# juanmc2005/diart

Hardware: NVIDIA H100
Metric: audio-seconds/sec (real-time factor) at 5s/0.5s step, batch 256 (higher is better)
Workload: dtype f32

## Files before the change

diart_b200/_lib.py:

```python
from __future__ import annotations

import ctypes as C
import os
from typing import Dict, Optional

import numpy as np
import torch

_HERE = os.path.dirname(os.path.abspath(__file__))
LIB_PATH = os.path.join(_HERE, "libdiartb200.so")

_lib: Optional[C.CDLL] = None


class DgTensor(C.Structure):
    _fields_ = [("name", C.c_char_p), ("data", C.c_void_p), ("numel", C.c_int64)]


_P = C.c_void_p
SIGNATURES = {
    "dg_last_error": (C.c_char_p, []),
    "dg_version": (C.c_int, []),
    "dg_launch_count": (C.c_int64, []),
    "dg_profile_enable": (C.c_int, [C.c_int]),
    "dg_profile_report": (C.c_int, [C.c_char_p, C.c_int]),
    "dg_selftest_gemm_tc": (C.c_int, [C.c_int, C.c_int, C.c_int, C.c_int, C.c_int, C.c_int, C.POINTER(C.c_float),
                                      C.POINTER(C.c_float)]),
    "dg_selftest_gemm_tc_grid": (C.c_int, [C.c_int, C.c_int, C.c_int, C.c_int, C.c_int, C.c_int, C.POINTER(C.c_int)]),
    "dg_selftest_gemm_tc_bounds": (C.c_int, [C.c_int, C.c_int, C.c_int, C.c_int, C.POINTER(C.c_int), C.POINTER(C.c_int),
                                             C.POINTER(C.c_int)]),
    "dg_selftest_wgmma_row_shift": (C.c_int, [C.c_int, C.POINTER(C.c_uint)]),
    "dg_selftest_gemm_tc_halo": (C.c_int, [C.c_int, C.c_int, C.c_int, C.c_int, C.c_int, C.c_int, C.POINTER(C.c_int),
                                           C.POINTER(C.c_int)]),
    "dg_selftest_split_f16_host": (C.c_int, [_P, C.c_longlong, _P, _P]),
    "dg_seg_create": (C.c_int, [C.POINTER(DgTensor), C.c_int, C.c_int, C.POINTER(_P)]),
    "dg_seg_dims": (C.c_int, [_P, C.c_int, C.POINTER(C.c_int), C.POINTER(C.c_int)]),
    "dg_seg_set_powerset": (C.c_int, [_P, C.c_int, C.c_int]),
    "dg_seg_forward": (C.c_int, [_P, _P, C.c_int, C.c_int, _P, _P]),
    "dg_seg_destroy": (C.c_int, [_P]),
    "dg_emb_create": (C.c_int, [C.POINTER(DgTensor), C.c_int, C.c_int, C.c_int, C.POINTER(_P)]),
    "dg_emb_dims": (C.c_int, [_P, C.c_int, C.POINTER(C.c_int), C.POINTER(C.c_int)]),
    "dg_emb_forward": (C.c_int, [_P, _P, _P, C.c_int, C.c_int, C.c_int, C.c_int, C.c_int, C.c_float, _P, _P]),
    "dg_emb_forward_rows": (C.c_int, [_P, _P, _P, C.c_int, C.c_int, C.c_int, _P, _P]),
    "dg_emb_destroy": (C.c_int, [_P]),
    "dg_emb_debug_trunk": (C.c_int, [_P, _P, C.c_int, C.c_int, C.c_int, _P, C.c_int64, _P]),
    "dg_seg_debug_stage": (C.c_int, [_P, _P, C.c_int, C.c_int, C.c_int, C.c_int, _P, C.c_int64, _P]),
    "dg_emb_debug_stage": (C.c_int, [_P, _P, _P, C.c_int, C.c_int, C.c_int, C.c_int, C.c_int, C.c_int, _P, C.c_int64, _P]),
    "dg_selftest_sinc_filters_host": (C.c_int, [_P, _P, _P]),
    "dg_osp": (C.c_int, [_P, C.c_int, C.c_int, C.c_int, C.c_float, C.c_float, C.c_int, _P, _P]),
    "dg_normalize_embeddings": (C.c_int, [_P, C.c_int, C.c_int, C.c_float, _P, _P]),
    "dg_cluster_create": (C.c_int, [C.c_int, C.c_int, C.c_double, C.c_double, C.c_double, C.c_int, C.POINTER(_P)]),
    "dg_cluster_set_metric": (C.c_int, [_P, C.c_int]),
    "dg_cluster_step": (C.c_int, [_P, _P, _P, C.c_int, C.c_int, C.c_int, _P, _P, _P]),
    "dg_cluster_reset": (C.c_int, [_P]),
    "dg_cluster_get_state": (C.c_int, [_P, _P, _P, C.POINTER(C.c_int)]),
    "dg_cluster_set_state": (C.c_int, [_P, _P, _P, C.c_int]),
# ... 143 lines not shown
```

diart_b200/csrc/api.cu:

```cuda
#include <math.h>
#include <stdlib.h>
#include <string.h>

#include <map>
#include <sstream>
#include <vector>

#include "host.cuh"

namespace dg {

static thread_local std::string g_err;
std::atomic<long long> g_launches{0};
thread_local int g_sm_limit = 0;
void set_error(const std::string& msg) { g_err = msg; }

struct ProfRec {
  std::string name;
  cudaEvent_t a, b;
};
static bool g_prof = false;
static std::vector<ProfRec> g_recs;
static const bool g_trace = getenv("DG_TRACE_LAUNCHES") && getenv("DG_TRACE_LAUNCHES")[0] == '1';
ProfScope::ProfScope(const char* name_, cudaStream_t st_) : on(g_prof), st(st_), a(nullptr), b(nullptr), name(name_) {
// ... 347 lines not shown
  }
  std::vector<unsigned char> first, cur;
  *equal = 1;
  for (int run = 0; run < 3; run++) {
    DG_CUDA(cudaMemset(dF.p, 0, f32_bytes + 4));
    DG_CUDA(cudaMemset(dOh.p, 0, plane_bytes + 4));
    DG_CUDA(cudaMemset(dOl.p, 0, plane_bytes + 4));
    DG_CUDA(cudaMemset(dPart.p, 0, part_bytes + 4));
    {
      SmLimit cap(run == 1 ? 3 : 0);
      if ((rc = launch_gemm_tc(run == 2 ? ref : t, nullptr))) return rc;
    }
    DG_CUDA(cudaDeviceSynchronize());
    cur.resize(f32_bytes + 2 * plane_bytes + part_bytes);
    DG_CUDA(cudaMemcpy(cur.data(), dF.p, f32_bytes, cudaMemcpyDeviceToHost));
    DG_CUDA(cudaMemcpy(cur.data() + f32_bytes, dOh.p, plane_bytes, cudaMemcpyDeviceToHost));
    DG_CUDA(cudaMemcpy(cur.data() + f32_bytes + plane_bytes, dOl.p, plane_bytes, cudaMemcpyDeviceToHost));
    DG_CUDA(cudaMemcpy(cur.data() + f32_bytes + 2 * plane_bytes, dPart.p, part_bytes, cudaMemcpyDeviceToHost));
    if (run == 0)
      first.swap(cur);
    else if (cur != first)
      *equal = 0;
  }
  return DG_OK;
}

extern "C" int dg_selftest_gemm_tc_bounds(int M, int Cin, int N, int epi, int* outside_unchanged, int* equal, int* refused) {
  const bool planes = epi == 1;
  if (M < 1 || Cin < 64 || Cin % 64 || N < 1 || N % (planes ? 32 : 4) || epi < 0 || epi > 2 || !outside_unchanged || !equal ||
      !refused) {
    set_error("dg_selftest_gemm_tc_bounds: bad arguments");
    return DG_EINVAL;
  }
  const int npad = N <= 64 && epi == 0 ? 64 : (N + 127) / 128 * 128, esize = planes ? 2 : 4;
  const int ldc = N + 40;
  const long long rows = (long long)M + 130;
  uint32_t seed = 4242u;
  auto rnd = [&]() {
    seed = seed * 1664525u + 1013904223u;
    return ((seed >> 8) & 0xFFFF) / 65536.f - 0.5f;
  };
  std::vector<float> A((size_t)M * Cin), Wnk((size_t)N * Cin), bias(N), bsc(N), bsh(N);
  for (auto& v : A) v = 2.f * rnd();
  for (auto& v : Wnk) v = 0.25f * rnd();
  for (int n = 0; n < N; n++) {
    bias[n] = rnd();
// ... 59 lines not shown
```

diart_b200/csrc/dg_common.cuh:

```cuda
#pragma once
#include <cuda_runtime.h>
#include <stdint.h>
#include <stdio.h>

#include <atomic>
#include <string>
#include <vector>

namespace dg {

void set_error(const std::string& msg);
extern std::atomic<long long> g_launches;
extern thread_local int g_sm_limit;
inline int usable_sms() {
  int dev = 0, sms = 132;
  cudaGetDevice(&dev);
  cudaDeviceGetAttribute(&sms, cudaDevAttrMultiProcessorCount, dev);
  return (g_sm_limit > 0 && g_sm_limit < sms) ? g_sm_limit : sms;
}

#define DG_CUDA(expr)                                                                   \
  do {                                                                                  \
    cudaError_t _e = (expr);                                                            \
    if (_e != cudaSuccess) {                                                            \
// ... 100 lines not shown
  float* out_f32;
  void* out_hi;
  void* out_lo;
  int ldc;
  int epi;
  const char* tag;
  const int* tap_off;
  int Wp, Hp, Wop, Hop, stride2, relu;
  const void* res_hi;
  const void* res_lo;
  const float* pool_w;
  float* pool_part;
  int pool_item_rows, pool_K;
  int pool3_T, pool3_tile_rows;
  int tap_boxes;
};
inline int gemm_tc_pool3_tile_rows(int item_rows) {
  for (int t = 126; t >= 96; t -= 3)
    if (item_rows % t == 0) return t;
  return 0;
}
int launch_gemm_tc(const TcGemm& g, cudaStream_t st);
bool gemm_tc_halo(const TcGemm& g);
int selftest_wgmma_row_shift(int base_offset_mode, unsigned* ok_shifts);
int launch_split_ex(const float* x, long long rows_out, int C, int ld_in, int ld_out, int pool, int item_rows,
                    const float* sc, const float* sh, void* hi, void* lo, cudaStream_t st, const int* skip_flag = nullptr);
void split_weights_host(const float* w, int N, int Npad, int K, uint16_t* hi, uint16_t* lo, float scale = 1.f);
float weight_plane_scale(const float* w, size_t n);
uint16_t host_f32_to_h16(float f);
float host_h16_to_f32(uint16_t h);
int sinc_tc_rows_per_item(const Geom& g);
size_t sinc_tc_plane_elems(int B, const Geom& g);
void sinc_tc_pack_filters(const float* filt, uint16_t* planes );
void sinc_tc_affine_consts(const float* filt, float beta, float* cf);
int launch_sinc_prep(const float* wav, const float* mean, const float* rstd, int B, const Geom& g, void* planes_hi,
                     void* planes_lo, cudaStream_t st, const int* skip_flag = nullptr);
int launch_sinc0_tc(float gamma, const float* cf_dev, const void* w_planes, int B, const Geom& g, const void* planes_hi,
                    const void* planes_lo, float* p0, cudaStream_t st, const int* skip_flag = nullptr);
struct SincStreamGeom {
  int Ls;
  int P;
  int rows;
  size_t plane;
};
SincStreamGeom sinc_stream_geom(int B, const Geom& g, int hop);
int launch_overlap_check(const float* wav, int B, int S, int hop, int* flag, cudaStream_t st);
// ... 143 lines not shown
```

diart_b200/csrc/gemm_tc.cu:

```cuda
#include <cuda.h>
#include <cuda_bf16.h>
#include <math.h>
#include <stdlib.h>
#include <string.h>

#include <algorithm>
#include <map>
#include <mutex>
#include <string>
#include <utility>
#include <vector>

#include "dg_common.cuh"
#include "tc_ptx.cuh"

namespace dg {

constexpr int TC_BM = 128, TC_BK = 32, TC_THREADS = 384;
constexpr int TC_SMEM_MAX = 227 * 1024;

struct TcArgs {
  long long M;
  int N;
  int m_tiles, n_tiles;
// ... 3 lines not shown
  const float* bn_shift;
  float* out_f32;
  __nv_bfloat16* out_hi;
  __nv_bfloat16* out_lo;
  int ldc;
  float acc_scale;
  int tap_off[9];
  int Wp, Hp, Wop, Hop, stride2, relu;
  const __nv_bfloat16* res_hi;
  const __nv_bfloat16* res_lo;
  const float* pool_w;
  float* pool_part;
  int pool_item_rows, pool_K;
  int tile_rows, pool3_T;
  unsigned* tile_ctr;
  int halo_rows;
  int cin;
  int wblocks;
  int halo_bytes;
  int op_bytes;
};

enum TcEpi { TC_BIAS_F32 = 0, TC_LEAKY_BN_SPLIT = 1, TC_LEAKY_BN_F32 = 2, TC_CONV2D = 3, TC_POOL = 4, TC_MAXPOOL3 = 5 };

__host__ __device__ constexpr bool tc_pooling(int epi) { return epi == TC_POOL || epi == TC_MAXPOOL3; }
__host__ __device__ constexpr bool tc_box_store(int epi) { return epi == TC_BIAS_F32 || epi == TC_LEAKY_BN_SPLIT || epi == TC_LEAKY_BN_F32; }

template <int BN>
struct TcSmem {
  static constexpr int A_BYTES = TC_BM * TC_BK * 2;
  static constexpr int W_BYTES = BN * TC_BK * 2;
  static constexpr int STAGE_BYTES = 2 * A_BYTES + 2 * W_BYTES;
  static constexpr int W_STAGE_BYTES = 2 * W_BYTES;
  static constexpr int NSTAGE = BN == 128 ? 4 : 6;
  static constexpr int NSTAGE_HALO = BN == 128 ? 5 : 6;
  __host__ static int halo_bytes(int cin, int rows) { return (2 * ((cin + 31) / 32) * rows * 64 + 1023) / 1024 * 1024; }
  __host__ static int halo_op_bytes(int cin, int rows) { return 2 * halo_bytes(cin, rows) + NSTAGE_HALO * W_STAGE_BYTES; }
  static constexpr int BAR_BYTES = 256;
  static constexpr int PARAM_FLOATS = 3 * BN;
  static constexpr int CHUNK_W = 64;
  static constexpr int CHUNK_FLOATS = CHUNK_W / 32 * TC_BM * 33;
  __host__ __device__ static constexpr int extra_floats(int epi) { return epi == TC_POOL ? 128 * 4 + 4 * 2 * 8 * 32 : (epi == TC_MAXPOOL3 ? 4 * 2 * 2 * 32 : 0); }
  __host__ __device__ static constexpr int consumer_floats(int epi) { return PARAM_FLOATS + (tc_pooling(epi) ? CHUNK_FLOATS + extra_floats(epi) : 0); }
  static constexpr int ACC_LD = BN + 4;
  static constexpr int BOX_BYTES = TC_BM * 128;
  __host__ __device__ static constexpr int stage_tile_bytes(int epi) {
    return tc_pooling(epi) ? 0 : (epi == TC_CONV2D ? TC_BM * ACC_LD * 4 : TC_BM * BN * 4);
  }
  __host__ __device__ static constexpr int total(int epi, int op_bytes = NSTAGE * STAGE_BYTES) {
    return op_bytes + stage_tile_bytes(epi) + BAR_BYTES + 2 * consumer_floats(epi) * 4 + 1024;
  }
};
static_assert(TcSmem<128>::total(TC_POOL) <= TC_SMEM_MAX && TcSmem<64>::total(TC_MAXPOOL3) <= TC_SMEM_MAX &&
              TcSmem<128>::total(TC_CONV2D) <= TC_SMEM_MAX && TcSmem<64>::total(TC_CONV2D) <= TC_SMEM_MAX &&
              TcSmem<32>::total(TC_CONV2D) <= TC_SMEM_MAX && TcSmem<128>::total(TC_BIAS_F32) <= TC_SMEM_MAX,
              "gemm_tc: shared memory");

template <int BN, int EPI>
__device__ __forceinline__ void tc_stage_params(const TcArgs& a, float* params, int bar, int n0, int et) {
  named_sync(bar, 128);
  for (int i = et; i < BN; i += 128) {
// ... 272 lines not shown
                }
              }
            }
#pragma unroll
            for (int sg = 0; sg < 2; sg++) {
              stg[((rg * 2 + sg) * 2 + 0) * 32 + col] = s1[sg];
              stg[((rg * 2 + sg) * 2 + 1) * 32 + col] = s2[sg];
            }
          }
          named_sync(bar, 128);
          {
            const int col = et & 31, q = et >> 5, sg = q >> 1, j = q & 1, n = n0 + c + col;
            const float tot = ((stg[((0 * 2 + sg) * 2 + j) * 32 + col] + stg[((1 * 2 + sg) * 2 + j) * 32 + col]) +
                               stg[((2 * 2 + sg) * 2 + j) * 32 + col]) + stg[((3 * 2 + sg) * 2 + j) * 32 + col];
            if (n < a.N) a.pool_part[(((size_t)mt * 2 + sg) * 2 + j) * a.N + n] = tot;
          }
          named_sync(bar, 128);
          continue;
        }
      }
    }
}

template <int BN, int EPI, bool HALO>
__global__ void __launch_bounds__(TC_THREADS, 1)
gemm_tc_kernel(const __grid_constant__ CUtensorMap tmA_hi, const __grid_constant__ CUtensorMap tmA_lo,
               const __grid_constant__ CUtensorMap tmW_hi, const __grid_constant__ CUtensorMap tmW_lo,
               const __grid_constant__ CUtensorMap tmC0, const __grid_constant__ CUtensorMap tmC1, TcArgs a) {
  using S = TcSmem<BN>;
  constexpr bool POOLING = tc_pooling(EPI);
  constexpr int NSTAGE = HALO ? S::NSTAGE_HALO : S::NSTAGE;
  extern __shared__ unsigned char smem_raw[];
  unsigned char* smem = reinterpret_cast<unsigned char*>((reinterpret_cast<uintptr_t>(smem_raw) + 1023) & ~uintptr_t(1023));
  unsigned char* ring = HALO ? smem + 2 * a.halo_bytes : smem;
  constexpr int RING_STAGE = HALO ? S::W_STAGE_BYTES : S::STAGE_BYTES;
  unsigned char* tile_s = smem + a.op_bytes;
  uint64_t* bars = reinterpret_cast<uint64_t*>(tile_s + S::stage_tile_bytes(EPI));
  uint64_t* full = bars;
  uint64_t* empty = bars + NSTAGE;
  uint64_t* tile_full = bars + 2 * NSTAGE;
  uint64_t* tile_empty = tile_full + 2;
  uint64_t* halo_full = tile_empty + 2;
  uint64_t* halo_empty = halo_full + 2;
  volatile int* tile_idx = reinterpret_cast<volatile int*>(halo_empty + 2);
  float* cons = reinterpret_cast<float*>(reinterpret_cast<unsigned char*>(bars) + S::BAR_BYTES);

  const int warp = __shfl_sync(0xffffffffu, (int)(threadIdx.x >> 5), 0), lane = threadIdx.x & 31;
  const int wg = warp >> 2;
  const int num_tiles = a.m_tiles * a.n_tiles;
  const int kblocks = HALO ? a.wblocks : a.KW * a.cin_blocks;
  const int halo_box = a.halo_rows * 64, halo_cb = (a.cin + 31) / 32;

  if (threadIdx.x == 0) {
    for (int s = 0; s < NSTAGE; s++) {
      mbar_init(&full[s], 1);
      mbar_init(&empty[s], 1);
    }
    for (int c = 0; c < 2; c++) {
      mbar_init(&tile_full[c], 1);
      mbar_init(&tile_empty[c], 128);
      mbar_init(&halo_full[c], 1);
      mbar_init(&halo_empty[c], 1);
    }
    asm volatile("fence.mbarrier_init.release.cluster;" ::: "memory");
  }
  __syncthreads();

  if (wg == 0) {
    setmaxnreg_dec<HALO ? 48 : 40>();
    if (threadIdx.x == 0) {
      int stage = 0, phase = 0, next = 0;
      bool halo_next = false;
      for (int i = 0, tile = blockIdx.x;; i++) {
        const int c = i & 1;
        mbar_wait(&tile_empty[c], ((i >> 1) & 1) ^ 1);
        if (tile >= num_tiles) {
          tile_idx[c] = -1;
          mbar_arrive(&tile_full[c]);
          mbar_wait(&tile_empty[c ^ 1], (((i + 1) >> 1) & 1) ^ 1);
          tile_idx[c ^ 1] = -2;
          mbar_arrive(&tile_full[c ^ 1]);
          break;
        }
        tile_idx[c] = tile;
        mbar_arrive(&tile_full[c]);
        const int mt = tile / a.n_tiles, nt = tile - mt * a.n_tiles;
        const int m0 = mt * (EPI == TC_MAXPOOL3 ? a.tile_rows : TC_BM), n0 = nt * BN;
        if constexpr (HALO) {
          auto load_halo = [&](int cc, int r0) {
            unsigned char* hs = smem + cc * a.halo_bytes;
            mbar_expect_tx(&halo_full[cc], 2 * halo_cb * halo_box);
            for (int cb = 0; cb < halo_cb; cb++) {
              tma_load_2d(hs + cb * halo_box, &tmA_hi, cb * TC_BK, r0, &halo_full[cc]);
              tma_load_2d(hs + (halo_cb + cb) * halo_box, &tmA_lo, cb * TC_BK, r0, &halo_full[cc]);
            }
          };
          if (!halo_next) {
            mbar_wait(&halo_empty[c], ((i >> 1) & 1) ^ 1);
            load_halo(c, m0);
          }
          halo_next = false;
          next = POOLING ? (int)gridDim.x + (int)atomicAdd(&a.tile_ctr[0], 1u) : tile + (int)gridDim.x;
          const int next_m0 = next / a.n_tiles * (EPI == TC_MAXPOOL3 ? a.tile_rows : TC_BM);
          const uint32_t next_par = (((i + 1) >> 1) & 1) ^ 1;
          for (int kb = 0; kb < kblocks; kb++) {
            const long long t0 = clock64();
            for (;;) {
              if (!halo_next && next < num_tiles && mbar_test_wait(&halo_empty[c ^ 1], next_par)) {
                load_halo(c ^ 1, next_m0);
                halo_next = true;
              }
              if (mbar_test_wait(&empty[stage], phase ^ 1)) break;
              if (clock64() - t0 > 4000000000LL) __trap();
            }
            unsigned char* st = ring + stage * RING_STAGE;
            mbar_expect_tx(&full[stage], S::W_STAGE_BYTES);
            tma_load_2d(st, &tmW_hi, kb * TC_BK, n0, &full[stage]);
            tma_load_2d(st + S::W_BYTES, &tmW_lo, kb * TC_BK, n0, &full[stage]);
            if (++stage == NSTAGE) {
              stage = 0;
              phase ^= 1;
            }
          }
        }
        for (int j = 0; j < (HALO ? 0 : a.KW); j++) {
          for (int cb = 0; cb < a.cin_blocks; cb++) {
            mbar_wait(&empty[stage], phase ^ 1);
            unsigned char* st = smem + stage * S::STAGE_BYTES;
            mbar_expect_tx(&full[stage], S::STAGE_BYTES);
            const int kcol = (j * a.cin_blocks + cb) * TC_BK;
            tma_load_2d(st, &tmA_hi, cb * TC_BK, m0 + a.tap_off[j], &full[stage]);
            tma_load_2d(st + S::A_BYTES, &tmA_lo, cb * TC_BK, m0 + a.tap_off[j], &full[stage]);
            tma_load_2d(st + 2 * S::A_BYTES, &tmW_hi, kcol, n0, &full[stage]);
            tma_load_2d(st + 2 * S::A_BYTES + S::W_BYTES, &tmW_lo, kcol, n0, &full[stage]);
            if (++stage == NSTAGE) {
              stage = 0;
              phase ^= 1;
            }
          }
        }
        if (!HALO) next = POOLING ? (int)gridDim.x + (int)atomicAdd(&a.tile_ctr[0], 1u) : tile + (int)gridDim.x;
        tile = next;
      }
      if (POOLING) {
        __threadfence();
        if (atomicAdd(&a.tile_ctr[1], 1u) == gridDim.x - 1) {
          atomicExch(&a.tile_ctr[0], 0u);
          atomicExch(&a.tile_ctr[1], 0u);
        }
      }
    }
    return;
  }
  setmaxnreg_inc<HALO ? 224 : 232>();
  const int c = wg - 1, quad = warp & 3, et = threadIdx.x - 128 * wg;
  float* params = cons + c * S::consumer_floats(EPI);
  float* chunk = params + S::PARAM_FLOATS;
  float* pool_stage = chunk + S::CHUNK_FLOATS;
  const int bar = 1 + c, turn = 3 + c, turn_other = 3 + (c ^ 1), acc_free = 5 + c, acc_free_other = 5 + (c ^ 1);
  if (c == 1) {
    named_arrive(3, 256);
    if (!POOLING) named_arrive(5, 256);
  }
  for (int n = 0;; n++) {
    mbar_wait(&tile_full[c], n & 1);
    const int tile = tile_idx[c];
    mbar_arrive(&tile_empty[c]);
    if (tc_box_store(EPI) && tile >= 0 && (a.n_tiles > 1 || n == 0))
      tc_stage_params<BN, EPI>(a, params, bar, (tile - tile / a.n_tiles * a.n_tiles) * BN, et);
    named_sync(turn, 256);
    if (tile < 0) {
      if (tile == -1) {
        named_arrive(turn_other, 256);
        if (!POOLING) named_sync(acc_free, 256);
      }
      break;
    }
    const int pos = (2 * n + c) * kblocks;
    int stage = pos % NSTAGE, phase = (pos / NSTAGE) & 1;
    float acc[2][BN / 2];
#pragma unroll
    for (int i = 0; i < BN / 2; i++) acc[0][i] = acc[1][i] = 0.f;
    uint32_t htap = 0;
    int hch = 0;
    if constexpr (HALO) mbar_wait(&halo_full[c], n & 1);
    const uint32_t hs = smem_u32(smem + c * a.halo_bytes);
    for (int kb = 0; kb < kblocks; kb++) {
      mbar_wait(&full[stage], phase);
      const uint32_t sa = smem_u32(ring + stage * RING_STAGE);
      const uint32_t sw = HALO ? sa : sa + 2 * S::A_BYTES;
      const uint64_t w_hi = wg_desc_sw64(sw), w_lo = wg_desc_sw64(sw + S::W_BYTES);
      constexpr uint64_t HALF = (uint64_t)((64 * TC_BK * 2) >> 4);
      wg_fence_acc(acc[0]);
      wg_fence_acc(acc[1]);
      wg_fence();
#pragma unroll
      for (int ks = 0; ks < TC_BK / 16; ks++) {
        const uint64_t adv = (uint64_t)((ks * 32) >> 4);
        uint64_t a_hi, a_lo;
        if constexpr (HALO) {
          const uint32_t aa = hs + (uint32_t)(hch >> 5) * halo_box + (uint32_t)(hch & 31) * 2 + htap;
          a_hi = wg_desc_sw64(aa);
          a_lo = wg_desc_sw64(aa + halo_cb * halo_box);
          hch += 16;
          const bool next_tap = hch == a.cin;
          hch = next_tap ? 0 : hch;
          htap += next_tap ? a.dil * 64 : 0;
        } else {
          a_hi = wg_desc_sw64(sa) + adv;
          a_lo = wg_desc_sw64(sa + S::A_BYTES) + adv;
        }
#pragma unroll
        for (int h = 0; h < 2; h++) {
          wgmma_ss<BN>(acc[h], a_lo + h * HALF, w_hi + adv, (kb | ks) != 0);
          wgmma_ss<BN>(acc[h], a_hi + h * HALF, w_lo + adv, 1);
          wgmma_ss<BN>(acc[h], a_hi + h * HALF, w_hi + adv, 1);
        }
      }
      wg_commit();
      wg_wait<1>();
      wg_fence_acc(acc[0]);
      wg_fence_acc(acc[1]);
      if (kb > 0 && et == 0) mbar_arrive(&empty[stage == 0 ? NSTAGE - 1 : stage - 1]);
      if (++stage == NSTAGE) {
        stage = 0;
        phase ^= 1;
      }
    }
    named_arrive(turn_other, 256);
    wg_wait<0>();
    wg_fence_acc(acc[0]);
    wg_fence_acc(acc[1]);
    if (et == 0) mbar_arrive(&empty[stage == 0 ? NSTAGE - 1 : stage - 1]);
    if (HALO && et == 0) mbar_arrive(&halo_empty[c]);
    const int mt = tile / a.n_tiles, nt = tile - mt * a.n_tiles;
    const bool stage_params = a.n_tiles > 1 || n == 0;
    if constexpr (POOLING) {
      tc_pool_epilogue_tile<BN, EPI>(a, params, chunk, pool_stage, acc, bar, mt, nt * BN, quad, lane, et, stage_params);
    } else if constexpr (EPI == TC_CONV2D) {
      float* acc_s = reinterpret_cast<float*>(tile_s);
      named_sync(acc_free, 256);
#pragma unroll
      for (int h = 0; h < 2; h++) {
        const int r0 = 64 * h + 16 * quad + (lane >> 2);
#pragma unroll
        for (int j = 0; j < BN / 8; j++) {
          const int col = 8 * j + 2 * (lane & 3);
          *reinterpret_cast<float2*>(acc_s + r0 * S::ACC_LD + col) = make_float2(acc[h][4 * j], acc[h][4 * j + 1]);
          *reinterpret_cast<float2*>(acc_s + (r0 + 8) * S::ACC_LD + col) = make_float2(acc[h][4 * j + 2], acc[h][4 * j + 3]);
        }
      }
      named_sync(bar, 128);
      if (stage_params) tc_stage_params<BN, EPI>(a, params, bar, nt * BN, et);
      tc_conv2d_epilogue_tile<BN>(a, params, acc_s + et * S::ACC_LD, mt, nt * BN, quad, lane);
      named_arrive(acc_free_other, 256);
    } else {
      named_sync(acc_free, 256);
// ... 77 lines not shown
  }
  void* base = nullptr;
  if (cudaGetSymbolAddress(&base, g_tc_tile_ctr) != cudaSuccess) {
    set_error("gemm_tc: cannot address the tile counters");
    return nullptr;
  }
  return static_cast<unsigned*>(base) + 2 * slot;
}

static int tc_bn(const TcGemm& g) { return g.epi == TC_MAXPOOL3 || (g.Npad == 64 && g.epi == TC_BIAS_F32) ? 64 : 128; }
static int tc_halo_rows(const TcGemm& g) {
  return (TC_BM + (g.KW - ((g.KW * g.Cin) % 32 ? 0 : 1)) * g.dil + 7) / 8 * 8;
}
template <int BN>
static int tc_halo_smem(const TcGemm& g) { return TcSmem<BN>::total(g.epi, TcSmem<BN>::halo_op_bytes(g.Cin, tc_halo_rows(g))); }

bool gemm_tc_halo(const TcGemm& g) {
  if (g.tap_boxes || g.epi == TC_CONV2D || g.tap_off || g.KW < 2 || g.dil < 1 || g.Cin % 16 || g.Cin > 128 ||
      tc_halo_rows(g) > 256)
    return false;
  return (tc_bn(g) == 64 ? tc_halo_smem<64>(g) : tc_halo_smem<128>(g)) <= TC_SMEM_MAX;
}

static int tc_setup(const TcGemm& g, int bn, int epi, bool halo, CUtensorMap* maps, TcArgs& a) {
  const int Ktot = g.KW * g.Cin, bk = TC_BK, a_rows = halo ? tc_halo_rows(g) : TC_BM;
  if (make_map(&maps[0], g.A_hi, g.Mtot, g.Cin, g.lda, bk, a_rows) || make_map(&maps[1], g.A_lo, g.Mtot, g.Cin, g.lda, bk, a_rows) ||
      make_map(&maps[2], g.W_hi, g.Npad, Ktot, Ktot, bk, bn) || make_map(&maps[3], g.W_lo, g.Npad, Ktot, Ktot, bk, bn))
    return -2;
  memset(&maps[4], 0, 2 * sizeof(CUtensorMap));
  if (epi == TC_LEAKY_BN_SPLIT) {
    if (make_map(&maps[4], g.out_hi, g.M, g.N, g.ldc, 64, TC_BM) || make_map(&maps[5], g.out_lo, g.M, g.N, g.ldc, 64, TC_BM))
      return -2;
  } else if (tc_box_store(epi)) {
    if (make_map(&maps[4], g.out_f32, g.M, g.N, g.ldc, 32, TC_BM, true)) return -2;
  }
  a = TcArgs{};
  a.M = g.M; a.N = g.N; a.n_tiles = (g.N + bn - 1) / bn;
  a.tile_rows = epi == TC_MAXPOOL3 ? g.pool3_tile_rows : TC_BM;
  a.pool3_T = g.pool3_T;
  a.m_tiles = (int)((g.M + a.tile_rows - 1) / a.tile_rows);
  a.KW = g.KW; a.dil = g.dil; a.cin_blocks = g.Cin / bk;
  a.bias = g.bias; a.bn_scale = g.bn_scale; a.bn_shift = g.bn_shift;
  a.out_f32 = g.out_f32; a.out_hi = reinterpret_cast<__nv_bfloat16*>(g.out_hi);
  a.out_lo = reinterpret_cast<__nv_bfloat16*>(g.out_lo); a.ldc = g.ldc;
  a.acc_scale = g.w_scale > 0.f ? 1.f / g.w_scale : 1.f;
  for (int j = 0; j < 9; j++) a.tap_off[j] = j < g.KW ? (g.tap_off ? g.tap_off[j] : j * g.dil) : 0;
  a.Wp = g.Wp; a.Hp = g.Hp; a.Wop = g.Wop; a.Hop = g.Hop; a.stride2 = g.stride2; a.relu = g.relu;
  a.res_hi = reinterpret_cast<const __nv_bfloat16*>(g.res_hi);
  a.res_lo = reinterpret_cast<const __nv_bfloat16*>(g.res_lo);
  a.pool_w = g.pool_w; a.pool_part = g.pool_part; a.pool_item_rows = g.pool_item_rows; a.pool_K = g.pool_K;
  a.cin = g.Cin;
  if (halo) {
    a.halo_rows = a_rows;
    a.wblocks = (Ktot + bk - 1) / bk;
    a.halo_bytes = bn == 64 ? TcSmem<64>::halo_bytes(g.Cin, a_rows) : TcSmem<128>::halo_bytes(g.Cin, a_rows);
    a.op_bytes = bn == 64 ? TcSmem<64>::halo_op_bytes(g.Cin, a_rows) : TcSmem<128>::halo_op_bytes(g.Cin, a_rows);
  } else {
    a.op_bytes = bn == 128 ? TcSmem<128>::NSTAGE * TcSmem<128>::STAGE_BYTES
                           : (bn == 64 ? TcSmem<64>::NSTAGE * TcSmem<64>::STAGE_BYTES : TcSmem<32>::NSTAGE * TcSmem<32>::STAGE_BYTES);
  }
  return 0;
}

static int tc_grid(const TcArgs& a) {
  const int sms = usable_sms();
  const int tiles = a.m_tiles * a.n_tiles;
  return tiles < sms ? tiles : sms;
}

template <int BN, int EPI, bool HALO>
static int launch_tc(const TcGemm& g, cudaStream_t st) {
  using S = TcSmem<BN>;
  CUtensorMap m[6];
  TcArgs a;
  if (tc_setup(g, BN, EPI, HALO, m, a)) return -2;
  if (tc_pooling(EPI) && !(a.tile_ctr = tile_counter(st))) return -2;
  auto kern = gemm_tc_kernel<BN, EPI, HALO>;
  static bool attr_done[64] = {};
  if (first_use_on_device(attr_done))
    DG_CUDA(cudaFuncSetAttribute(kern, cudaFuncAttributeMaxDynamicSharedMemorySize, HALO ? TC_SMEM_MAX : S::total(EPI)));
  kern<<<tc_grid(a), TC_THREADS, S::total(EPI, a.op_bytes), st>>>(m[0], m[1], m[2], m[3], m[4], m[5], a);
  DG_LAUNCHED();
  return 0;
}

template <int BN, int EPI>
static int launch_tc(const TcGemm& g, cudaStream_t st) {
  return gemm_tc_halo(g) ? launch_tc<BN, EPI, true>(g, st) : launch_tc<BN, EPI, false>(g, st);
}

int launch_gemm_tc(const TcGemm& g, cudaStream_t st) {
  ProfScope _ps(g.tag ? g.tag : "gemm_tc", st);
  if (g.Cin % (gemm_tc_halo(g) ? 16 : 64) || g.lda % 8 || g.ldc % (g.epi == TC_LEAKY_BN_SPLIT ? 8 : 4) ||
      (g.Npad % 128 && g.Npad != 64 && g.Npad != 32) || g.KW < 1 || g.KW > 9) {
    set_error("gemm_tc: Cin must be a multiple of 64 (a Conv1d of 2..9 taps over at most 128 channels whose tile halo fits "
              "in shared memory, e.g. Cin 80: a multiple of 16), A pitch a multiple of 8, output pitch a multiple of 4 "
              "(8 for 16-bit planes), padded N 32, 64 or a multiple of 128, at most 9 taps");
    return -1;
  }
  if (g.epi == TC_LEAKY_BN_SPLIT && g.N % 32) {
    set_error("gemm_tc (planes): N must be a multiple of 32");
    return -1;
  }
  if (tc_box_store(g.epi)) {
    const bool planes = g.epi == TC_LEAKY_BN_SPLIT;
    const uintptr_t base = planes ? ((uintptr_t)g.out_hi | (uintptr_t)g.out_lo) : (uintptr_t)g.out_f32;
    if (!base || (planes && (!g.out_hi || !g.out_lo)) || base % 16 || g.ldc < g.N || g.M >= (1LL << 31)) {
      set_error("gemm_tc: the output needs a 16-byte aligned base, a pitch of at least N and fewer than 2^31 rows");
      return -1;
    }
  }
  if (g.epi == TC_CONV2D) {
    if (g.ldc % 32 || g.N % 32 || g.Wp < 3 || g.Hp < 3 || (!g.out_hi && !g.out_f32) || g.M >= (1LL << 31)) {
      set_error("gemm_tc (conv2d): channel counts must be multiples of 32");
      return -1;
    }
    if (g.Npad == 32) return launch_tc<32, TC_CONV2D, false>(g, st);
    if (g.Npad == 64) return launch_tc<64, TC_CONV2D, false>(g, st);
    return launch_tc<128, TC_CONV2D, false>(g, st);
  }
  if (g.epi == TC_POOL) {
    if (g.Npad % 128 || !g.pool_w || !g.pool_part || g.pool_K < 1 || g.pool_K > 4 || g.pool_item_rows < TC_BM) {
      set_error("gemm_tc (pool): needs 128-wide tiles, 1..4 speakers and items of at least 128 rows");
      return -1;
    }
    return launch_tc<128, TC_POOL>(g, st);
  }
  if (g.epi == TC_MAXPOOL3) {
    if (g.Npad != 64 || !g.out_f32 || !g.pool_part || g.pool3_T < 1 || g.pool3_tile_rows < 3 || g.pool3_tile_rows > 126 ||
        g.pool3_tile_rows % 3 || g.pool_item_rows % g.pool3_tile_rows || g.M % g.pool_item_rows) {
      set_error("gemm_tc (maxpool3): needs 64 output channels and tiles of 3..126 rows (a multiple of 3) that divide the item");
      return -1;
    }
    return launch_tc<64, TC_MAXPOOL3>(g, st);
  }
  if (g.Npad == 64 && g.epi == TC_BIAS_F32) return launch_tc<64, TC_BIAS_F32>(g, st);
  switch (g.epi) {
    case TC_BIAS_F32:
      return launch_tc<128, TC_BIAS_F32>(g, st);
    case TC_LEAKY_BN_SPLIT:
      return launch_tc<128, TC_LEAKY_BN_SPLIT>(g, st);
    default:
// ... 198 lines not shown
```

include/diart_b200.h:

```cpp
#ifndef DIART_B200_H
#define DIART_B200_H

#include <stddef.h>
#include <stdint.h>

#ifdef __cplusplus
extern "C" {
#endif

#define DG_OK 0
#define DG_EINVAL (-1)
#define DG_ECUDA (-2)
#define DG_EWEIGHT (-3)
#define DG_ENCCL (-4)

typedef struct dg_tensor {
  const char* name;
  const float* data;
  int64_t numel;
} dg_tensor;

typedef struct dg_seg dg_seg;
typedef struct dg_emb dg_emb;
typedef struct dg_cluster dg_cluster;
// ... 151 lines not shown
int dg_selftest_multi_frames_host(int slots, int max_wps, int out_chunk, int out_step, int n_rates, const int32_t* rates,
                                  int n_ops, const int32_t* ops, int32_t* result, int64_t* records, int cap, int* n_records);
int dg_selftest_multi_staging_host(int slots, int C, int n_ops, const int32_t* ops, const float* samples_host, int32_t* result,
                                   float* rings_host);
int dg_multi_create_vad(dg_seg* seg, int chunk_samples, int step_samples, int max_streams, int max_windows_per_stream,
                        double tau, int num_windows, const double* hamming_host, dg_multi** out);

typedef struct dg_resample dg_resample;
int dg_resample_create(int orig_rate, int new_rate, const float* taps_host, int width, int device, dg_resample** out);
int64_t dg_resample_out_len(const dg_resample* h, int64_t num_samples);
int dg_resample_forward(dg_resample* h, const float* in_dev, int B, int64_t L, float* out_dev, void* stream);
int dg_resample_destroy(dg_resample* h);
int dg_stream_create_resampled(int chunk_samples, int step_samples, dg_resample* rs, int max_windows, int device,
                               dg_stream** out);
int dg_stream_crop_host(dg_stream* h, int n, const int64_t* ranges_host, float* out_host);

int64_t dg_launch_count(void);
int dg_profile_enable(int enable);
int dg_selftest_gemm_tc(int M, int Cin, int KW, int dil, int N, int epi, float* max_abs_diff, float* out_rms);
int dg_selftest_gemm_tc_grid(int M, int Cin, int KW, int dil, int N, int epi, int* equal);
int dg_selftest_gemm_tc_bounds(int M, int Cin, int N, int epi, int* outside_unchanged, int* equal, int* refused);
int dg_selftest_wgmma_row_shift(int base_offset_mode, unsigned* ok_shifts);
int dg_selftest_gemm_tc_halo(int M, int Cin, int KW, int dil, int N, int epi, int* equal, int* halo);
int dg_selftest_split_f16_host(const float* x, long long n, unsigned short* hi, unsigned short* lo);
int dg_selftest_sinc_filters_host(const float* low_hz, const float* band_hz, float* filters);
int dg_profile_report(char* buf, int cap);

int dg_cluster_record_len(const dg_cluster* h);
int dg_cluster_export_delta(dg_cluster* h, double* record_dev, void* stream);
int dg_cluster_merge(dg_cluster* h, const double* records_dev , int world, int rank,
                     int32_t* maps_dev , int n_maps, void* stream);
int dg_pipeline_identity_export(dg_pipeline* h, double* record_dev, void* stream);
int dg_pipeline_identity_merge(dg_pipeline* h, const double* records_dev, int world, int rank, void* stream);

#ifdef __cplusplus
}
#endif
#endif
```

Measured before the change: 23040.

## Add per-channel-block halo A-loading mode to TMA/WGMMA conv GEMM

Adds a third A-operand mode for the tensor-core conv GEMM, used when the full halo tile does not fit in shared memory. Each 32-channel block is loaded once as a halo tile covering all taps into a three-slot ring, and only the weight tiles are streamed per tap. This replaces reloading the A box for every tap, cutting A-side TMA traffic and shared-memory fill per K step. It also switches to an atomic tile counter when the SM count is capped, and adds a selftest comparing the new mode against tap-box loading. The extra barriers and slots add complexity and more shared memory.

```diff
diff --git a/diart_b200/_lib.py b/diart_b200/_lib.py
--- a/diart_b200/_lib.py
+++ b/diart_b200/_lib.py
@@ -32,6 +32,8 @@
     "dg_selftest_wgmma_row_shift": (C.c_int, [C.c_int, C.POINTER(C.c_uint)]),
     "dg_selftest_gemm_tc_halo": (C.c_int, [C.c_int, C.c_int, C.c_int, C.c_int, C.c_int, C.c_int, C.POINTER(C.c_int),
                                            C.POINTER(C.c_int)]),
+    "dg_selftest_gemm_tc_modes": (C.c_int, [C.c_int, C.c_int, C.c_int, C.c_int, C.c_int, C.c_int, C.c_int, C.POINTER(C.c_int),
+                                            C.POINTER(C.c_float), C.POINTER(C.c_float), C.POINTER(C.c_int)]),
     "dg_selftest_split_f16_host": (C.c_int, [_P, C.c_longlong, _P, _P]),
     "dg_seg_create": (C.c_int, [C.POINTER(DgTensor), C.c_int, C.c_int, C.POINTER(_P)]),
     "dg_seg_dims": (C.c_int, [_P, C.c_int, C.POINTER(C.c_int), C.POINTER(C.c_int)]),
diff --git a/diart_b200/csrc/api.cu b/diart_b200/csrc/api.cu
--- a/diart_b200/csrc/api.cu
+++ b/diart_b200/csrc/api.cu
@@ -393,6 +393,98 @@
     else if (cur != first)
       *equal = 0;
   }
+  return DG_OK;
+}
+
+extern "C" int dg_selftest_gemm_tc_modes(int M, int Cin, int KW, int dil, int N, int epi, int shift, int* mode,
+                                         float* max_abs_diff, float* sum_abs, int* shift_equal) {
+  if (M < 1 || Cin < 64 || Cin % 64 || KW < 1 || KW > 9 || dil < 1 || N < 1 || N % 4 || epi < 0 || epi > 2 ||
+      (epi == 1 && N % 32) || shift < 0 || !mode || !max_abs_diff || !sum_abs || !shift_equal) {
+    set_error("dg_selftest_gemm_tc_modes: bad arguments");
+    return DG_EINVAL;
+  }
+  const int K = KW * Cin, npad = N == 64 ? 64 : (N + 127) / 128 * 128;
+  const long long Ms = (long long)M + shift;
+  uint32_t seed = 5151u;
+  auto rnd = [&]() {
+    seed = seed * 1664525u + 1013904223u;
+    return ((seed >> 8) & 0xFFFF) / 65536.f - 0.5f;
+  };
+  std::vector<float> A((size_t)Ms * Cin), Aabs(A.size()), Wnk((size_t)N * K), Wabs_kn((size_t)K * N), bias(N), bsc(N), bsh(N);
+  for (auto& v : A) v = 2.f * rnd();
+  for (auto& v : Wnk) v = 0.25f * rnd();
+  for (int n = 0; n < N; n++) {
+    bias[n] = rnd();
+    bsc[n] = 1.f + rnd();
+    bsh[n] = rnd();
+  }
+  for (size_t i = 0; i < A.size(); i++) Aabs[i] = fabsf(A[i]);
+  for (int n = 0; n < N; n++)
+    for (int k = 0; k < K; k++) Wabs_kn[(size_t)k * N + n] = fabsf(Wnk[(size_t)n * K + k]);
+  const bool planes = epi == 1;
+  const size_t out_bytes = (size_t)Ms * N * (planes ? 2 : 4);
+  DevBuf dA, dAabs, dWabs, dB, dS, dH, dAh, dAl, dSum, dO[3], dOl[3];
+  WeightPlanes dW;
+  if (upload(dA, A) || upload(dAabs, Aabs) || upload(dWabs, Wabs_kn) || upload(dB, bias) || upload(dS, bsc) || upload(dH, bsh) ||
+      upload_split(dW, Wnk, N, npad, K))
+    return DG_ECUDA;
+  if (dAh.ensure((size_t)Ms * Cin * 2) || dAl.ensure((size_t)Ms * Cin * 2) || dSum.ensure((size_t)M * N * 4)) return DG_ECUDA;
+  for (int r = 0; r < 3; r++)
+    if (dO[r].ensure(out_bytes) || dOl[r].ensure(out_bytes)) return DG_ECUDA;
+  int rc;
+  if ((rc = launch_split_ex(dA.as<float>(), Ms, Cin, Cin, Cin, 0, 1, nullptr, nullptr, dAh.p, dAl.p, nullptr))) return rc;
+  const size_t a_off = (size_t)shift * Cin * 2;
+  TcGemm t{};
+  t.A_hi = static_cast<char*>(dAh.p) + a_off; t.A_lo = static_cast<char*>(dAl.p) + a_off; t.lda = Cin; t.Cin = Cin;
+  t.KW = KW; t.dil = dil; t.Mtot = M; t.M = M; t.N = N; t.bias = dB.as<float>(); t.bn_scale = dS.as<float>();
+  t.bn_shift = dH.as<float>(); t.ldc = N; t.epi = epi; t.tag = "selftest_tc_modes";
+  if ((rc = set_weights(t, dW))) return rc;
+  *mode = gemm_tc_halo(t) ? 1 : (gemm_tc_cb_halo(t) ? 2 : 0);
+  TcGemm boxes = t, shifted = t;
+  boxes.tap_boxes = 1;
+  shifted.A_hi = dAh.p; shifted.A_lo = dAl.p; shifted.Mtot = shifted.M = Ms;
+  const TcGemm* runs[3] = {&t, &boxes, &shifted};
+  for (int r = 0; r < 3; r++) {
+    TcGemm g = *runs[r];
+    g.out_f32 = planes ? nullptr : dO[r].as<float>();
+    g.out_hi = planes ? dO[r].p : nullptr;
+    g.out_lo = planes ? dOl[r].p : nullptr;
+    if ((rc = launch_gemm_tc(g, nullptr))) return rc;
+  }
+  GemmArgs s{};
+  s.A = dAabs.as<float>() + (size_t)shift * Cin; s.lda = Cin; s.Cin = Cin; s.KW = KW; s.dil = dil; s.Mtot = M; s.M = M;
+  s.W = dWabs.as<float>(); s.ldw = N; s.N = N; s.C = dSum.as<float>(); s.ldc = N; s.epi = EPI_BIAS; s.tag = "selftest_simt";
+  if ((rc = launch_gemm(s, nullptr))) return rc;
+  DG_CUDA(cudaDeviceSynchronize());
+  std::vector<unsigned char> o[3], ol[3];
+  for (int r = 0; r < 3; r++) {
+    const size_t bytes = (r == 2 ? (size_t)Ms : (size_t)M) * N * (planes ? 2 : 4);
+    o[r].resize(bytes);
+    DG_CUDA(cudaMemcpy(o[r].data(), dO[r].p, bytes, cudaMemcpyDeviceToHost));
+    if (planes) {
+      ol[r].resize(bytes);
+      DG_CUDA(cudaMemcpy(ol[r].data(), dOl[r].p, bytes, cudaMemcpyDeviceToHost));
+    }
+  }
+  auto value = [&](int r, size_t i) {
+    if (!planes) return (double)reinterpret_cast<const float*>(o[r].data())[i];
+    return (double)host_h16_to_f32(reinterpret_cast<const uint16_t*>(o[r].data())[i]) +
+           (double)host_h16_to_f32(reinterpret_cast<const uint16_t*>(ol[r].data())[i]);
+  };
+  std::vector<float> sums((size_t)M * N);
+  DG_CUDA(cudaMemcpy(sums.data(), dSum.p, sums.size() * 4, cudaMemcpyDeviceToHost));
+  double md = 0, ms = 0;
+  for (size_t i = 0; i < (size_t)M * N; i++) {
+    const double d = fabs(value(0, i) - value(1, i));
+    if (!(d <= md)) md = d;
+    const double sg = (double)sums[i] * (epi == 0 ? 1.0 : fabs((double)bsc[i % N]));
+    if (sg > ms) ms = sg;
+  }
+  *max_abs_diff = (float)md;
+  *sum_abs = (float)ms;
+  const size_t row_bytes = (size_t)N * (planes ? 2 : 4), skip = (size_t)shift * row_bytes;
+  *shift_equal = memcmp(o[0].data(), o[2].data() + skip, (size_t)M * row_bytes) == 0 &&
+                 (!planes || memcmp(ol[0].data(), ol[2].data() + skip, (size_t)M * row_bytes) == 0);
   return DG_OK;
 }
 
diff --git a/diart_b200/csrc/dg_common.cuh b/diart_b200/csrc/dg_common.cuh
--- a/diart_b200/csrc/dg_common.cuh
+++ b/diart_b200/csrc/dg_common.cuh
@@ -146,6 +146,7 @@
 }
 int launch_gemm_tc(const TcGemm& g, cudaStream_t st);
 bool gemm_tc_halo(const TcGemm& g);
+bool gemm_tc_cb_halo(const TcGemm& g);
 int selftest_wgmma_row_shift(int base_offset_mode, unsigned* ok_shifts);
 int launch_split_ex(const float* x, long long rows_out, int C, int ld_in, int ld_out, int pool, int item_rows,
                     const float* sc, const float* sh, void* hi, void* lo, cudaStream_t st, const int* skip_flag = nullptr);
diff --git a/diart_b200/csrc/gemm_tc.cu b/diart_b200/csrc/gemm_tc.cu
--- a/diart_b200/csrc/gemm_tc.cu
+++ b/diart_b200/csrc/gemm_tc.cu
@@ -49,6 +49,8 @@
 };
 
 enum TcEpi { TC_BIAS_F32 = 0, TC_LEAKY_BN_SPLIT = 1, TC_LEAKY_BN_F32 = 2, TC_CONV2D = 3, TC_POOL = 4, TC_MAXPOOL3 = 5 };
+enum TcAMode { TC_TAP_BOXES = 0, TC_HALO = 1, TC_CB_HALO = 2 };
+constexpr int TC_CB_SLOTS = 3;
 
 __host__ __device__ constexpr bool tc_pooling(int epi) { return epi == TC_POOL || epi == TC_MAXPOOL3; }
 __host__ __device__ constexpr bool tc_box_store(int epi) { return epi == TC_BIAS_F32 || epi == TC_LEAKY_BN_SPLIT || epi == TC_LEAKY_BN_F32; }
@@ -63,7 +65,10 @@
   static constexpr int NSTAGE_HALO = BN == 128 ? 5 : 6;
   __host__ static int halo_bytes(int cin, int rows) { return (2 * ((cin + 31) / 32) * rows * 64 + 1023) / 1024 * 1024; }
   __host__ static int halo_op_bytes(int cin, int rows) { return 2 * halo_bytes(cin, rows) + NSTAGE_HALO * W_STAGE_BYTES; }
+  static constexpr int NSTAGE_CB = 6;
+  __host__ static int cb_op_bytes(int rows) { return TC_CB_SLOTS * halo_bytes(32, rows) + NSTAGE_CB * W_STAGE_BYTES; }
   static constexpr int BAR_BYTES = 256;
+  static_assert((2 * 6 + 4 + 2 * TC_CB_SLOTS) * 8 + 8 <= BAR_BYTES, "gemm_tc: barrier block");
   static constexpr int PARAM_FLOATS = 3 * BN;
   static constexpr int CHUNK_W = 64;
   static constexpr int CHUNK_FLOATS = CHUNK_W / 32 * TC_BM * 33;
@@ -382,18 +387,19 @@
     }
 }
 
-template <int BN, int EPI, bool HALO>
+template <int BN, int EPI, int AMODE>
 __global__ void __launch_bounds__(TC_THREADS, 1)
 gemm_tc_kernel(const __grid_constant__ CUtensorMap tmA_hi, const __grid_constant__ CUtensorMap tmA_lo,
                const __grid_constant__ CUtensorMap tmW_hi, const __grid_constant__ CUtensorMap tmW_lo,
                const __grid_constant__ CUtensorMap tmC0, const __grid_constant__ CUtensorMap tmC1, TcArgs a) {
   using S = TcSmem<BN>;
   constexpr bool POOLING = tc_pooling(EPI);
-  constexpr int NSTAGE = HALO ? S::NSTAGE_HALO : S::NSTAGE;
+  constexpr bool HALO = AMODE == TC_HALO, CB_HALO = AMODE == TC_CB_HALO;
+  constexpr int NSTAGE = HALO ? S::NSTAGE_HALO : (CB_HALO ? S::NSTAGE_CB : S::NSTAGE);
   extern __shared__ unsigned char smem_raw[];
   unsigned char* smem = reinterpret_cast<unsigned char*>((reinterpret_cast<uintptr_t>(smem_raw) + 1023) & ~uintptr_t(1023));
-  unsigned char* ring = HALO ? smem + 2 * a.halo_bytes : smem;
-  constexpr int RING_STAGE = HALO ? S::W_STAGE_BYTES : S::STAGE_BYTES;
+  unsigned char* ring = smem + (HALO ? 2 : (CB_HALO ? TC_CB_SLOTS : 0)) * a.halo_bytes;
+  constexpr int RING_STAGE = AMODE != TC_TAP_BOXES ? S::W_STAGE_BYTES : S::STAGE_BYTES;
   unsigned char* tile_s = smem + a.op_bytes;
   uint64_t* bars = reinterpret_cast<uint64_t*>(tile_s + S::stage_tile_bytes(EPI));
   uint64_t* full = bars;
@@ -401,8 +407,8 @@
   uint64_t* tile_full = bars + 2 * NSTAGE;
   uint64_t* tile_empty = tile_full + 2;
   uint64_t* halo_full = tile_empty + 2;
-  uint64_t* halo_empty = halo_full + 2;
-  volatile int* tile_idx = reinterpret_cast<volatile int*>(halo_empty + 2);
+  uint64_t* halo_empty = halo_full + TC_CB_SLOTS;
+  volatile int* tile_idx = reinterpret_cast<volatile int*>(halo_empty + TC_CB_SLOTS);
   float* cons = reinterpret_cast<float*>(reinterpret_cast<unsigned char*>(bars) + S::BAR_BYTES);
 
   const int warp = __shfl_sync(0xffffffffu, (int)(threadIdx.x >> 5), 0), lane = threadIdx.x & 31;
@@ -419,17 +425,20 @@
     for (int c = 0; c < 2; c++) {
       mbar_init(&tile_full[c], 1);
       mbar_init(&tile_empty[c], 128);
-      mbar_init(&halo_full[c], 1);
-      mbar_init(&halo_empty[c], 1);
+    }
+    for (int s = 0; s < TC_CB_SLOTS; s++) {
+      mbar_init(&halo_full[s], 1);
+      mbar_init(&halo_empty[s], 1);
     }
     asm volatile("fence.mbarrier_init.release.cluster;" ::: "memory");
   }
   __syncthreads();
 
   if (wg == 0) {
-    setmaxnreg_dec<HALO ? 48 : 40>();
+    setmaxnreg_dec<AMODE != TC_TAP_BOXES ? 48 : 40>();
     if (threadIdx.x == 0) {
       int stage = 0, phase = 0, next = 0;
+      int astage = 0, aphase = 0;
       bool halo_next = false;
       for (int i = 0, tile = blockIdx.x;; i++) {
         const int c = i & 1;
@@ -460,7 +469,7 @@
             load_halo(c, m0);
           }
           halo_next = false;
-          next = POOLING ? (int)gridDim.x + (int)atomicAdd(&a.tile_ctr[0], 1u) : tile + (int)gridDim.x;
+          next = a.tile_ctr ? (int)gridDim.x + (int)atomicAdd(&a.tile_ctr[0], 1u) : tile + (int)gridDim.x;
           const int next_m0 = next / a.n_tiles * (EPI == TC_MAXPOOL3 ? a.tile_rows : TC_BM);
           const uint32_t next_par = (((i + 1) >> 1) & 1) ^ 1;
           for (int kb = 0; kb < kblocks; kb++) {
@@ -483,7 +492,32 @@
             }
           }
         }
-        for (int j = 0; j < (HALO ? 0 : a.KW); j++) {
+        if constexpr (CB_HALO) {
+          for (int cb = 0; cb < a.cin_blocks; cb++) {
+            mbar_wait(&halo_empty[astage], aphase ^ 1);
+            unsigned char* as = smem + astage * a.halo_bytes;
+            mbar_expect_tx(&halo_full[astage], 2 * halo_box);
+            tma_load_2d(as, &tmA_hi, cb * TC_BK, m0, &halo_full[astage]);
+            tma_load_2d(as + halo_box, &tmA_lo, cb * TC_BK, m0, &halo_full[astage]);
+            if (++astage == TC_CB_SLOTS) {
+              astage = 0;
+              aphase ^= 1;
+            }
+            for (int j = 0; j < a.KW; j++) {
+              mbar_wait(&empty[stage], phase ^ 1);
+              unsigned char* st = ring + stage * RING_STAGE;
+              mbar_expect_tx(&full[stage], S::W_STAGE_BYTES);
+              const int kcol = j * a.cin + cb * TC_BK;
+              tma_load_2d(st, &tmW_hi, kcol, n0, &full[stage]);
+              tma_load_2d(st + S::W_BYTES, &tmW_lo, kcol, n0, &full[stage]);
+              if (++stage == NSTAGE) {
+                stage = 0;
+                phase ^= 1;
+              }
+            }
+          }
+        }
+        for (int j = 0; j < (AMODE == TC_TAP_BOXES ? a.KW : 0); j++) {
           for (int cb = 0; cb < a.cin_blocks; cb++) {
             mbar_wait(&empty[stage], phase ^ 1);
             unsigned char* st = smem + stage * S::STAGE_BYTES;
@@ -499,10 +533,10 @@
             }
           }
         }
-        if (!HALO) next = POOLING ? (int)gridDim.x + (int)atomicAdd(&a.tile_ctr[0], 1u) : tile + (int)gridDim.x;
+        if (!HALO) next = a.tile_ctr ? (int)gridDim.x + (int)atomicAdd(&a.tile_ctr[0], 1u) : tile + (int)gridDim.x;
         tile = next;
       }
-      if (POOLING) {
+      if (a.tile_ctr) {
         __threadfence();
         if (atomicAdd(&a.tile_ctr[1], 1u) == gridDim.x - 1) {
           atomicExch(&a.tile_ctr[0], 0u);
@@ -512,7 +546,7 @@
     }
     return;
   }
-  setmaxnreg_inc<HALO ? 224 : 232>();
+  setmaxnreg_inc<AMODE != TC_TAP_BOXES ? 224 : 232>();
   const int c = wg - 1, quad = warp & 3, et = threadIdx.x - 128 * wg;
   float* params = cons + c * S::consumer_floats(EPI);
   float* chunk = params + S::PARAM_FLOATS;
@@ -538,6 +572,8 @@
     }
     const int pos = (2 * n + c) * kblocks;
     int stage = pos % NSTAGE, phase = (pos / NSTAGE) & 1;
+    const int apos = (2 * n + c) * a.cin_blocks;
+    int astage = apos % TC_CB_SLOTS, aphase = (apos / TC_CB_SLOTS) & 1, tap = 0;
     float acc[2][BN / 2];
 #pragma unroll
     for (int i = 0; i < BN / 2; i++) acc[0][i] = acc[1][i] = 0.f;
@@ -546,9 +582,10 @@
     if constexpr (HALO) mbar_wait(&halo_full[c], n & 1);
     const uint32_t hs = smem_u32(smem + c * a.halo_bytes);
     for (int kb = 0; kb < kblocks; kb++) {
+      if constexpr (CB_HALO) mbar_wait(&halo_full[astage], aphase);
       mbar_wait(&full[stage], phase);
       const uint32_t sa = smem_u32(ring + stage * RING_STAGE);
-      const uint32_t sw = HALO ? sa : sa + 2 * S::A_BYTES;
+      const uint32_t sw = AMODE != TC_TAP_BOXES ? sa : sa + 2 * S::A_BYTES;
       const uint64_t w_hi = wg_desc_sw64(sw), w_lo = wg_desc_sw64(sw + S::W_BYTES);
       constexpr uint64_t HALF = (uint64_t)((64 * TC_BK * 2) >> 4);
       wg_fence_acc(acc[0]);
@@ -566,6 +603,10 @@
           const bool next_tap = hch == a.cin;
           hch = next_tap ? 0 : hch;
           htap += next_tap ? a.dil * 64 : 0;
+        } else if constexpr (CB_HALO) {
+          const uint32_t aa = smem_u32(smem + astage * a.halo_bytes) + (uint32_t)(tap * a.dil * 64 + ks * 32);
+          a_hi = wg_desc_sw64(aa);
+          a_lo = wg_desc_sw64(aa + halo_box);
         } else {
           a_hi = wg_desc_sw64(sa) + adv;
           a_lo = wg_desc_sw64(sa + S::A_BYTES) + adv;
@@ -586,6 +627,16 @@
         stage = 0;
         phase ^= 1;
       }
+      if constexpr (CB_HALO) {
+        if (tap == 0 && kb > 0 && et == 0) mbar_arrive(&halo_empty[astage == 0 ? TC_CB_SLOTS - 1 : astage - 1]);
+        if (++tap == a.KW) {
+          tap = 0;
+          if (++astage == TC_CB_SLOTS) {
+            astage = 0;
+            aphase ^= 1;
+          }
+        }
+      }
     }
     named_arrive(turn_other, 256);
     wg_wait<0>();
@@ -593,6 +644,7 @@
     wg_fence_acc(acc[1]);
     if (et == 0) mbar_arrive(&empty[stage == 0 ? NSTAGE - 1 : stage - 1]);
     if (HALO && et == 0) mbar_arrive(&halo_empty[c]);
+    if (CB_HALO && et == 0) mbar_arrive(&halo_empty[astage == 0 ? TC_CB_SLOTS - 1 : astage - 1]);
     const int mt = tile / a.n_tiles, nt = tile - mt * a.n_tiles;
     const bool stage_params = a.n_tiles > 1 || n == 0;
     if constexpr (POOLING) {
@@ -716,8 +768,21 @@
   return (tc_bn(g) == 64 ? tc_halo_smem<64>(g) : tc_halo_smem<128>(g)) <= TC_SMEM_MAX;
 }
 
-static int tc_setup(const TcGemm& g, int bn, int epi, bool halo, CUtensorMap* maps, TcArgs& a) {
-  const int Ktot = g.KW * g.Cin, bk = TC_BK, a_rows = halo ? tc_halo_rows(g) : TC_BM;
+static int tc_cb_rows(const TcGemm& g) { return (TC_BM + (g.KW - 1) * g.dil + 7) / 8 * 8; }
+template <int BN>
+static int tc_cb_smem(const TcGemm& g) { return TcSmem<BN>::total(g.epi, TcSmem<BN>::cb_op_bytes(tc_cb_rows(g))); }
+
+bool gemm_tc_cb_halo(const TcGemm& g) {
+  if (g.tap_boxes || !tc_box_store(g.epi) || g.tap_off || g.KW < 2 || g.KW > 9 || g.dil < 1 || g.Cin % 32 ||
+      tc_cb_rows(g) > 256 || gemm_tc_halo(g))
+    return false;
+  return (tc_bn(g) == 64 ? tc_cb_smem<64>(g) : tc_cb_smem<128>(g)) <= TC_SMEM_MAX;
+}
+
+static int tc_setup(const TcGemm& g, int bn, int epi, int amode, CUtensorMap* maps, TcArgs& a) {
+  const bool halo = amode == TC_HALO;
+  const int Ktot = g.KW * g.Cin, bk = TC_BK;
+  const int a_rows = halo ? tc_halo_rows(g) : (amode == TC_CB_HALO ? tc_cb_rows(g) : TC_BM);
   if (make_map(&maps[0], g.A_hi, g.Mtot, g.Cin, g.lda, bk, a_rows) || make_map(&maps[1], g.A_lo, g.Mtot, g.Cin, g.lda, bk, a_rows) ||
       make_map(&maps[2], g.W_hi, g.Npad, Ktot, Ktot, bk, bn) || make_map(&maps[3], g.W_lo, g.Npad, Ktot, Ktot, bk, bn))
     return -2;
@@ -749,11 +814,22 @@
     a.wblocks = (Ktot + bk - 1) / bk;
     a.halo_bytes = bn == 64 ? TcSmem<64>::halo_bytes(g.Cin, a_rows) : TcSmem<128>::halo_bytes(g.Cin, a_rows);
     a.op_bytes = bn == 64 ? TcSmem<64>::halo_op_bytes(g.Cin, a_rows) : TcSmem<128>::halo_op_bytes(g.Cin, a_rows);
+  } else if (amode == TC_CB_HALO) {
+    a.halo_rows = a_rows;
+    a.halo_bytes = TcSmem<128>::halo_bytes(32, a_rows);
+    a.op_bytes = bn == 64 ? TcSmem<64>::cb_op_bytes(a_rows) : TcSmem<128>::cb_op_bytes(a_rows);
   } else {
     a.op_bytes = bn == 128 ? TcSmem<128>::NSTAGE * TcSmem<128>::STAGE_BYTES
                            : (bn == 64 ? TcSmem<64>::NSTAGE * TcSmem<64>::STAGE_BYTES : TcSmem<32>::NSTAGE * TcSmem<32>::STAGE_BYTES);
   }
   return 0;
+}
+
+static bool tc_capped() {
+  int dev = 0, sms = 0;
+  if (cudaGetDevice(&dev) != cudaSuccess || cudaDeviceGetAttribute(&sms, cudaDevAttrMultiProcessorCount, dev) != cudaSuccess)
+    return false;
+  return usable_sms() < sms;
 }
 
 static int tc_grid(const TcArgs& a) {
@@ -762,17 +838,18 @@
   return tiles < sms ? tiles : sms;
 }
 
-template <int BN, int EPI, bool HALO>
+template <int BN, int EPI, int AMODE>
 static int launch_tc(const TcGemm& g, cudaStream_t st) {
   using S = TcSmem<BN>;
   CUtensorMap m[6];
   TcArgs a;
-  if (tc_setup(g, BN, EPI, HALO, m, a)) return -2;
-  if (tc_pooling(EPI) && !(a.tile_ctr = tile_counter(st))) return -2;
-  auto kern = gemm_tc_kernel<BN, EPI, HALO>;
+  if (tc_setup(g, BN, EPI, AMODE, m, a)) return -2;
+  if ((tc_pooling(EPI) || tc_capped()) && !(a.tile_ctr = tile_counter(st))) return -2;
+  auto kern = gemm_tc_kernel<BN, EPI, AMODE>;
   static bool attr_done[64] = {};
   if (first_use_on_device(attr_done))
-    DG_CUDA(cudaFuncSetAttribute(kern, cudaFuncAttributeMaxDynamicSharedMemorySize, HALO ? TC_SMEM_MAX : S::total(EPI)));
+    DG_CUDA(cudaFuncSetAttribute(kern, cudaFuncAttributeMaxDynamicSharedMemorySize,
+                                 AMODE != TC_TAP_BOXES ? TC_SMEM_MAX : S::total(EPI)));
   kern<<<tc_grid(a), TC_THREADS, S::total(EPI, a.op_bytes), st>>>(m[0], m[1], m[2], m[3], m[4], m[5], a);
   DG_LAUNCHED();
   return 0;
@@ -780,7 +857,10 @@
 
 template <int BN, int EPI>
 static int launch_tc(const TcGemm& g, cudaStream_t st) {
-  return gemm_tc_halo(g) ? launch_tc<BN, EPI, true>(g, st) : launch_tc<BN, EPI, false>(g, st);
+  if (gemm_tc_halo(g)) return launch_tc<BN, EPI, TC_HALO>(g, st);
+  if constexpr (tc_box_store(EPI))
+    if (gemm_tc_cb_halo(g)) return launch_tc<BN, EPI, TC_CB_HALO>(g, st);
+  return launch_tc<BN, EPI, TC_TAP_BOXES>(g, st);
 }
 
 int launch_gemm_tc(const TcGemm& g, cudaStream_t st) {
@@ -809,9 +889,9 @@
       set_error("gemm_tc (conv2d): channel counts must be multiples of 32");
       return -1;
     }
-    if (g.Npad == 32) return launch_tc<32, TC_CONV2D, false>(g, st);
-    if (g.Npad == 64) return launch_tc<64, TC_CONV2D, false>(g, st);
-    return launch_tc<128, TC_CONV2D, false>(g, st);
+    if (g.Npad == 32) return launch_tc<32, TC_CONV2D, TC_TAP_BOXES>(g, st);
+    if (g.Npad == 64) return launch_tc<64, TC_CONV2D, TC_TAP_BOXES>(g, st);
+    return launch_tc<128, TC_CONV2D, TC_TAP_BOXES>(g, st);
   }
   if (g.epi == TC_POOL) {
     if (g.Npad % 128 || !g.pool_w || !g.pool_part || g.pool_K < 1 || g.pool_K > 4 || g.pool_item_rows < TC_BM) {
diff --git a/include/diart_b200.h b/include/diart_b200.h
--- a/include/diart_b200.h
+++ b/include/diart_b200.h
@@ -197,6 +197,8 @@
 int dg_selftest_gemm_tc_bounds(int M, int Cin, int N, int epi, int* outside_unchanged, int* equal, int* refused);
 int dg_selftest_wgmma_row_shift(int base_offset_mode, unsigned* ok_shifts);
 int dg_selftest_gemm_tc_halo(int M, int Cin, int KW, int dil, int N, int epi, int* equal, int* halo);
+int dg_selftest_gemm_tc_modes(int M, int Cin, int KW, int dil, int N, int epi, int shift, int* mode, float* max_abs_diff,
+                              float* sum_abs, int* shift_equal);
 int dg_selftest_split_f16_host(const float* x, long long n, unsigned short* hi, unsigned short* lo);
 int dg_selftest_sinc_filters_host(const float* low_hz, const float* band_hz, float* filters);
 int dg_profile_report(char* buf, int cap);
```

New measurement: 23980 (median of 6 runs). 4.1% higher.
